# cvxopt/cvxopt

Hardware: NVIDIA H100
Metric: kkt_factor_solve_gflops_fp64 (higher is better)
Workload: dtype f64

## Files before the change

cvxopt_b200/csrc/chol.cu:

```cuda
#include "common.cuh"
#include <cstdlib>

namespace cvxb {

namespace {

constexpr int PB = 8;
constexpr int SP = 12;
constexpr int LDM = NB + 4;
constexpr int POTF2_SMEM = (NB * LDM + NB * SP + 4 * 80) * 8;
constexpr int kGroup = 4;

template <int PAT>
__device__ __forceinline__ void sym_update(double (&acc)[4][8][2], const double *Ma, const double *Mb) {
#pragma unroll 2
    for (int kk = 0; kk < NB / 4; ++kk) {
        double a[4], bfr[8];
#pragma unroll
        for (int cf = 0; cf < 4; ++cf) a[cf] = -Ma[cf * 8 + kk * 4 * LDM];
#pragma unroll
        for (int rf = 0; rf < 8; ++rf) bfr[rf] = Mb[rf * 8 + kk * 4 * LDM];
#pragma unroll
        for (int mf = 0; mf < 2; ++mf)
#pragma unroll
            for (int rf = 0; rf < 8; ++rf) {
                if (PAT == 1 && rf < 2 * mf) continue;
                if (PAT == 2 && rf < 4 + 2 * mf) continue;
                dmma16x8x4(acc[2 * mf][rf][0], acc[2 * mf][rf][1], acc[2 * mf + 1][rf][0], acc[2 * mf + 1][rf][1],
                           a[2 * mf], a[2 * mf + 1], bfr[rf]);
            }
    }
}

__global__ void __launch_bounds__(256, 1)
potf2_inv_kernel(double *A, long long lda, int jb, double *inv, double *invT, int *info, int joff,
                 long long sA, long long sInv, const double *Tprev, long long ldt,
                 const double *invprev, unsigned long long *trace) {
    extern __shared__ __align__(16) double sm[];
    if (trace && threadIdx.x == 0) {
        unsigned long long t; asm volatile("mov.u64 %0, %%globaltimer;" : "=l"(t)); trace[0] = t;
    }
#define CVXB_STAMP(SLOT)                                                                    \
    if (trace && threadIdx.x == 0) {                                                        \
        unsigned long long t_; asm volatile("mov.u64 %0, %%globaltimer;" : "=l"(t_));       \
        trace[8 * 2048 + (SLOT)] = t_;                                                      \
    }
    A += (long long)blockIdx.x * sA; inv += (long long)blockIdx.x * sInv;
    invT += (long long)blockIdx.x * sInv; info += blockIdx.x;
    double *M = sm;
    double *P = M + NB * LDM;
    double *Dw = P + NB * SP;
    const int tid = threadIdx.x, lane = tid & 31, warp = tid >> 5;
    const int role = (0x72640531 >> (warp * 4)) & 7;
    const int wr = role & 1, wc = role >> 1;
    const int g4 = lane >> 2, t4 = lane & 3;

    double acc[4][8][2];
    if (Tprev != nullptr) {
#pragma unroll
        for (int cf = 0; cf < 4; ++cf)
#pragma unroll
            for (int rf = 0; rf < 8; ++rf) acc[cf][rf][0] = acc[cf][rf][1] = 0.0;
        const int kkmax = (wc + 1) * 8;
        {
            const bool v16 = ((ldt & 1) == 0) && ((reinterpret_cast<uintptr_t>(Tprev) & 15) == 0);
            if (v16) {
                for (int q = tid; q < NB * NB / 2; q += 256) {
                    const int c = q >> 6, r = (q & 63) * 2;
                    const int nb = (r + 1 < jb) ? 16 : (r < jb ? 8 : 0);
                    cp_async16(M + r + c * LDM, nb ? Tprev + r + (long long)c * ldt : Tprev, nb);
                }
            } else {
                for (int q = tid; q < NB * NB; q += 256) {
                    const int c = q >> 7, r = q & 127;
                    cp_async8(M + r + c * LDM, (r < jb) ? Tprev + r + (long long)c * ldt : Tprev, (r < jb) ? 8 : 0);
                }
            }
            cp_async_commit();
        }
        const double *ip = invprev + (wc * 32 + g4) + t4 * NB;
        double a0[4];
#pragma unroll
        for (int cf = 0; cf < 4; ++cf) a0[cf] = ip[cf * 8];
        cp_async_wait<0>();
        __syncthreads();
        const double *tq = M + (wr * 64 + g4) + t4 * LDM;
#pragma unroll 2
        for (int kk = 0; kk < kkmax; ++kk) {
            double a[4], bfr[8];
#pragma unroll
            for (int cf = 0; cf < 4; ++cf) a[cf] = a0[cf];
            if (kk + 1 < kkmax) {
#pragma unroll
                for (int cf = 0; cf < 4; ++cf) a0[cf] = ip[cf * 8 + (kk + 1) * 4 * NB];
            }
#pragma unroll
            for (int rf = 0; rf < 8; ++rf) bfr[rf] = tq[rf * 8 + kk * 4 * LDM];
#pragma unroll
            for (int mf = 0; mf < 2; ++mf)
#pragma unroll
                for (int rf = 0; rf < 8; ++rf)
                    dmma16x8x4(acc[2 * mf][rf][0], acc[2 * mf][rf][1], acc[2 * mf + 1][rf][0],
                               acc[2 * mf + 1][rf][1], a[2 * mf], a[2 * mf + 1], bfr[rf]);
        }
        __syncthreads();
#pragma unroll
        for (int cf = 0; cf < 4; ++cf)
#pragma unroll
            for (int rf = 0; rf < 8; ++rf)
#pragma unroll
                for (int e = 0; e < 2; ++e)
                    M[(wr * 64 + rf * 8 + t4 * 2 + e) + (wc * 32 + cf * 8 + g4) * LDM] = acc[cf][rf][e];
    }
    CVXB_STAMP(0)
#pragma unroll
    for (int cf = 0; cf < 4; ++cf)
#pragma unroll
        for (int rf = 0; rf < 8; ++rf)
#pragma unroll
            for (int e = 0; e < 2; ++e) {
                const int r = wr * 64 + rf * 8 + t4 * 2 + e, c = wc * 32 + cf * 8 + g4;
                double v = (r == c) ? 1.0 : 0.0;
                if (r < jb && c < jb && r >= c) v = A[r + (long long)c * lda];
                acc[cf][rf][e] = v;
            }
    __syncthreads();
    CVXB_STAMP(4)
    if (Tprev != nullptr) {
        const int d = wc - 2 * wr;
        const double *Ma = M + (wc * 32 + g4) + t4 * LDM;
        const double *Mb = M + (wr * 64 + g4) + t4 * LDM;
        if (d < 0) sym_update<0>(acc, Ma, Mb);
        else if (d == 0) sym_update<1>(acc, Ma, Mb);
        else if (d == 1) sym_update<2>(acc, Ma, Mb);
        __syncthreads();
    }
    CVXB_STAMP(1)
#pragma unroll 1
    for (int t = 0; t < NB / PB; ++t) {
      {
        const int c0 = t * PB;
        if (wc == (t >> 2)) {
#define CVXB_PUBLISH(CF)                                                          \
    _Pragma("unroll") for (int rf = 0; rf < 8; ++rf)                              \
        _Pragma("unroll") for (int e = 0; e < 2; ++e)                             \
            P[(wr * 64 + rf * 8 + t4 * 2 + e) * SP + g4] = acc[CF][rf][e];
            switch (t & 3) {
                case 0: CVXB_PUBLISH(0) break;
                case 1: CVXB_PUBLISH(1) break;
                case 2: CVXB_PUBLISH(2) break;
                default: CVXB_PUBLISH(3) break;
            }
#undef CVXB_PUBLISH
        }
        __syncthreads();
        if (warp == 0 && lane == 0) {
            double a[PB][PB];
#pragma unroll
            for (int i = 0; i < PB; ++i)
#pragma unroll
                for (int k = 0; k <= i; ++k) a[i][k] = P[(c0 + i) * SP + k];
            bool bad = false;
#pragma unroll
            for (int j = 0; j < PB; ++j) {
                const double piv = a[j][j];
                if (!(piv > 0.0) && !bad) {
                    atomicCAS(info, 0, joff + c0 + j + 1);
                    bad = true;
                }
                const double rs = rsqrt(piv);
                a[j][j] = piv * rs;
                Dw[64 + j] = rs;
#pragma unroll
                for (int i = j + 1; i < PB; ++i) a[i][j] *= rs;
#pragma unroll
                for (int k = j + 1; k < PB; ++k)
#pragma unroll
                    for (int i = k; i < PB; ++i) a[i][k] -= a[i][j] * a[k][j];
            }
#pragma unroll
            for (int i = 0; i < PB; ++i)
#pragma unroll
                for (int k = 0; k < PB; ++k) Dw[i * 8 + k] = (k <= i) ? a[i][k] : 0.0;
        }
        if (warp < 4) asm volatile("bar.sync 1, 128;" ::: "memory");
        if (warp < 4) {
            const double *D = Dw;
            const int r = warp * 32 + lane;
            double x[PB];
            if (r >= c0 + PB) {
#pragma unroll
                for (int j = 0; j < PB; ++j) x[j] = P[r * SP + j];
#pragma unroll
                for (int j = 0; j < PB; ++j) {
                    double v = x[j];
#pragma unroll
                    for (int k = 0; k < j; ++k) v -= x[k] * D[j * 8 + k];
                    x[j] = v * D[64 + j];
                }
            } else if (r >= c0) {
#pragma unroll
                for (int j = 0; j < PB; ++j) x[j] = (j <= r - c0) ? D[(r - c0) * 8 + j] : 0.0;
            } else {
#pragma unroll
                for (int j = 0; j < PB; ++j) x[j] = 0.0;
            }
#pragma unroll
            for (int j = 0; j < PB; ++j) P[r * SP + j] = x[j];
        }
        __syncthreads();
        if (wr * 8 + 7 > t && wc * 4 + 3 > t) {
            double a[4][2], bfr[8][2];
#pragma unroll
            for (int kk = 0; kk < 2; ++kk) {
#pragma unroll
                for (int cf = 0; cf < 4; ++cf) a[cf][kk] = -P[(wc * 32 + cf * 8 + g4) * SP + kk * 4 + t4];
#pragma unroll
                for (int rf = 0; rf < 8; ++rf) bfr[rf][kk] = P[(wr * 64 + rf * 8 + g4) * SP + kk * 4 + t4];
            }
#pragma unroll
            for (int mf = 0; mf < 2; ++mf) {
                if (wc * 4 + 2 * mf + 1 <= t) continue;
#pragma unroll
                for (int rf = 0; rf < 8; ++rf) {
                    dmma16x8x4(acc[2 * mf][rf][0], acc[2 * mf][rf][1], acc[2 * mf + 1][rf][0], acc[2 * mf + 1][rf][1],
                               a[2 * mf][0], a[2 * mf + 1][0], bfr[rf][0]);
                    dmma16x8x4(acc[2 * mf][rf][0], acc[2 * mf][rf][1], acc[2 * mf + 1][rf][0], acc[2 * mf + 1][rf][1],
                               a[2 * mf][1], a[2 * mf + 1][1], bfr[rf][1]);
                }
            }
        }
        for (int e = tid; e < NB * PB; e += 256) {
            const int r = e & (NB - 1), j = e >> 7;
            const double v = P[r * SP + j];
            M[r + (c0 + j) * LDM] = v;
            if (r >= c0 + j && r < jb && c0 + j < jb) A[r + (long long)(c0 + j) * lda] = v;
        }
        __syncthreads();
      }
    }

    CVXB_STAMP(2)
    {
        const int blk = warp * 2 + (lane >> 4);
        const int j = lane & 15;
        const int o = blk * PB;
        double x[PB];
        if (j < PB) {
#pragma unroll
            for (int i = 0; i < PB; ++i) {
                double v = (i == j) ? 1.0 : 0.0;
#pragma unroll
                for (int k = 0; k < i; ++k)
                    if (k >= j) v -= M[(o + i) + (o + k) * LDM] * x[k];
                x[i] = (i >= j) ? v / M[(o + i) + (o + i) * LDM] : 0.0;
            }
        }
        __syncwarp();
        if (j < PB) {
#pragma unroll
            for (int i = 0; i < PB; ++i) M[(o + i) + (o + j) * LDM] = x[i];
        }
    }
    __syncthreads();
    for (int s = PB; s < NB; s <<= 1) {
        const int sb = s / PB;
        const int tp = sb * sb;
        const int ntiles = (NB / (2 * s)) * tp;
#pragma unroll 1
        for (int phase = 0; phase < 2; ++phase) {
            for (int base = warp * 4; base < ntiles; base += 32) {
                double c[4][2];
                int oo[4], ti[4], tj[4];
#pragma unroll
                for (int u = 0; u < 4; ++u) {
                    const int idx = min(base + u, ntiles - 1);
                    const int pr = idx / tp, loc = idx - pr * tp;
                    ti[u] = loc % sb; tj[u] = loc / sb; oo[u] = pr * 2 * s;
                    c[u][0] = c[u][1] = 0.0;
                }
                for (int kb = 0; kb < sb; ++kb) {
#pragma unroll
                    for (int u = 0; u < 4; ++u) {
                        const bool live = phase == 0 ? (kb >= tj[u]) : (kb <= ti[u]);
                        if (!live) continue;
                        const int o = oo[u];
#pragma unroll
                        for (int kk = 0; kk < 2; ++kk) {
                            const int k = kb * 8 + kk * 4 + t4;
                            double af, bf;
                            if (phase == 0) {
                                af = M[(o + s + ti[u] * 8 + g4) + (o + k) * LDM];
                                bf = M[(o + k) + (o + tj[u] * 8 + g4) * LDM];
                            } else {
                                af = M[(o + s + ti[u] * 8 + g4) + (o + s + k) * LDM];
                                bf = M[(o + k) + (o + s + tj[u] * 8 + g4) * LDM];
                            }
                            dmma(c[u][0], c[u][1], af, bf);
                        }
                    }
                }
#pragma unroll
                for (int u = 0; u < 4; ++u) {
                    if (base + u >= ntiles) continue;
                    const int o = oo[u];
                    if (phase == 0) {
                        M[(o + ti[u] * 8 + g4) + (o + s + tj[u] * 8 + t4 * 2) * LDM] = c[u][0];
                        M[(o + ti[u] * 8 + g4) + (o + s + tj[u] * 8 + t4 * 2 + 1) * LDM] = c[u][1];
                    } else {
                        M[(o + s + ti[u] * 8 + g4) + (o + tj[u] * 8 + t4 * 2) * LDM] = -c[u][0];
                        M[(o + s + ti[u] * 8 + g4) + (o + tj[u] * 8 + t4 * 2 + 1) * LDM] = -c[u][1];
                    }
                }
            }
            __syncthreads();
        }
    }
    CVXB_STAMP(3)
    for (int e = tid; e < NB * NB; e += 256) {
        int i = e & (NB - 1), k = e >> 7;
        inv[e] = (i >= k) ? M[i + k * LDM] : 0.0;
        invT[e] = (k >= i) ? M[k + i * LDM] : 0.0;
    }
    if (trace && threadIdx.x == 0) {
        unsigned long long t; asm volatile("mov.u64 %0, %%globaltimer;" : "=l"(t)); trace[1] = t;
    }
}

constexpr int TR_CH = 32;
constexpr int TR_R = 5;
constexpr int TRSV_SMEM = (TR_R * NB * TR_CH + 4 * NB + 32 * 129) * 8;

template <bool TRANS, bool VEC>
__global__ void __launch_bounds__(256, 1)
trsv_kernel(int n, const double *__restrict__ L, long long ldl, const double *__restrict__ inv,
            const double *__restrict__ invT, double *b, int *flags, int epoch, long long sL,
            long long sInv, long long sb) {
    extern __shared__ __align__(16) double sm[];
    {
        const long long pb = blockIdx.y;
        L += pb * sL; inv += pb * sInv; invT += pb * sInv; b += pb * sb;
        flags += pb * ((n + NB - 1) / NB);
    }
    double *ring = sm;
    double *xs = ring + TR_R * NB * TR_CH;
    double *part = xs + NB;
    double *tvec = part + 2 * NB;
    double *part2 = tvec + NB;
    const int nblk = (n + NB - 1) / NB;
    const int tid = threadIdx.x, lane = tid & 31, warp = tid >> 5;
    const int bi = TRANS ? (nblk - 1 - (int)blockIdx.x) : (int)blockIdx.x;
    const int i0 = bi * NB;
    const int ni = min(NB, n - i0);
    const int r = tid & (NB - 1), half = tid >> 7;

    double ireg[64];
    {
        const double *ip = (TRANS ? invT : inv) + (long long)bi * NB * NB + r + (long long)(half * 64) * NB;
#pragma unroll
        for (int k = 0; k < 64; ++k) ireg[k] = ip[k * NB];
    }

    const double bown = (tid < ni) ? b[i0 + tid] : 0.0;
    const int nb_dep = TRANS ? (nblk - 1 - bi) : bi;
    const int nchunks = nb_dep * (NB / TR_CH);
    auto issue = [&](int q) {
        const int jj = q / (NB / TR_CH), cc = q % (NB / TR_CH);
        const int j = TRANS ? (nblk - 1 - jj) : jj;
        double *dst = ring + (q % TR_R) * (NB * TR_CH);
        const double *src;
        int nrows, ncols;
        if (!TRANS) { src = L + i0 + (long long)(j * NB + cc * TR_CH) * ldl; nrows = ni; ncols = TR_CH; }
        else { src = L + (long long)j * NB + (long long)(i0 + cc * TR_CH) * ldl; nrows = min(NB, n - j * NB); ncols = min(TR_CH, ni - cc * TR_CH); }
        if (VEC) {
#pragma unroll
            for (int it = 0; it < 8; ++it) {
                const int e = tid + it * 256;
                const int c = e >> 6, rr = (e & 63) * 2;
                const int rem = nrows - rr;
                const int bytes = (c < ncols) ? (rem >= 2 ? 16 : (rem == 1 ? 8 : 0)) : 0;
                cp_async16(dst + c * NB + rr, bytes ? (src + rr + (long long)c * ldl) : L, bytes);
            }
        } else {
#pragma unroll
            for (int it = 0; it < 16; ++it) {
                const int e = tid + it * 256;
                const int c = e >> 7, rr = e & 127;
                const int bytes = (c < ncols && rr < nrows) ? 8 : 0;
                cp_async8(dst + c * NB + rr, bytes ? (src + rr + (long long)c * ldl) : L, bytes);
            }
        }
    };
#pragma unroll
    for (int q = 0; q < TR_R - 1; ++q) {
        if (q < nchunks) issue(q);
        cp_async_commit();
    }

    double acc = 0.0;
    double accc[16];
#pragma unroll
    for (int q = 0; q < 16; ++q) accc[q] = 0.0;

    for (int jj = 0; jj < nb_dep; ++jj) {
        const int j = TRANS ? (nblk - 1 - jj) : jj;
        if (tid == 0) while (ld_acquire(flags + j) != epoch) { }
        __syncthreads();
        if (tid < NB) xs[tid] = (j * NB + tid < n) ? __ldcg(b + j * NB + tid) : 0.0;
#pragma unroll
        for (int cc = 0; cc < NB / TR_CH; ++cc) {
            const int q = jj * (NB / TR_CH) + cc;
            cp_async_wait<TR_R - 2>();
            __syncthreads();
            {
                const int nq = q + TR_R - 1;
                if (nq < nchunks) issue(nq);
                cp_async_commit();
            }
            const double *ch = ring + (q % TR_R) * (NB * TR_CH);
            if (!TRANS) {
#pragma unroll
                for (int c = 0; c < 16; ++c)
                    acc += ch[(half * 16 + c) * NB + r] * xs[cc * TR_CH + half * 16 + c];
            } else {
#pragma unroll
                for (int qc = 0; qc < 4; ++qc) {
                    const double *col = ch + (warp * 4 + qc) * NB;
                    double a = 0.0;
#pragma unroll
                    for (int rr = 0; rr < 4; ++rr) a += col[lane + rr * 32] * xs[lane + rr * 32];
                    accc[cc * 4 + qc] += a;
                }
            }
        }
    }
    cp_async_wait<0>();
    __syncthreads();
    if (!TRANS) {
        part[half * NB + r] = acc;
        __syncthreads();
        if (tid < NB) tvec[tid] = (tid < ni) ? (bown - part[tid] - part[NB + tid]) : 0.0;
        __syncthreads();
    } else {
#pragma unroll
        for (int q = 0; q < 16; ++q) {
            const int c = (q >> 2) * TR_CH + warp * 4 + (q & 3);
            part2[lane * 129 + c] = accc[q];
        }
        __syncthreads();
        if (tid < NB) {
            double sacc = 0.0;
#pragma unroll 8
            for (int l = 0; l < 32; ++l) sacc += part2[l * 129 + tid];
            tvec[tid] = (tid < ni) ? (bown - sacc) : 0.0;
        }
        __syncthreads();
    }
    double a2 = 0.0;
#pragma unroll
    for (int k = 0; k < 64; ++k) a2 += ireg[k] * tvec[half * 64 + k];
    part[half * NB + r] = a2;
    __syncthreads();
    if (tid < ni) b[i0 + tid] = part[tid] + part[NB + tid];
    __threadfence();
    __syncthreads();
    if (tid == 0) st_release(flags + bi, epoch);
}

std::atomic<int> g_trsv_epoch{0};

__global__ void __launch_bounds__(256)
transpose_panel_kernel(const double *__restrict__ W, long long ldw, int rows, double *__restrict__ WT, long long ldt) {
    __shared__ double t[32][33];
    const int r0 = blockIdx.x * 32, k0 = blockIdx.y * 32, tx = threadIdx.x, ty = threadIdx.y;
#pragma unroll
    for (int i = ty; i < 32; i += 8)
        if (r0 + tx < rows) t[i][tx] = W[r0 + tx + (long long)(k0 + i) * ldw];
    __syncthreads();
#pragma unroll
    for (int i = ty; i < 32; i += 8)
        if (r0 + i < rows) WT[k0 + tx + (long long)(r0 + i) * ldt] = t[tx][i];
}

}

int chol_work_create(CholWork &w) {
    int least = 0, greatest = 0;
    CVXB_CUDA(cudaDeviceGetStreamPriorityRange(&least, &greatest));
    CVXB_CUDA(cudaStreamCreateWithPriority(&w.panel_stream, cudaStreamNonBlocking, greatest));
    CVXB_CUDA(cudaStreamCreateWithPriority(&w.trsm_stream, cudaStreamNonBlocking, greatest));
    CVXB_CUDA(cudaStreamCreateWithPriority(&w.update_stream, cudaStreamNonBlocking, least));
    CVXB_CUDA(cudaStreamCreateWithPriority(&w.near_stream, cudaStreamNonBlocking, greatest));
    CVXB_CUDA(cudaEventCreateWithFlags(&w.ev_end_t, cudaEventDisableTiming));
    CVXB_CUDA(cudaEventCreateWithFlags(&w.ev_end_n, cudaEventDisableTiming));
    CVXB_CUDA(cudaEventCreateWithFlags(&w.ev_start, cudaEventDisableTiming));
    CVXB_CUDA(cudaEventCreateWithFlags(&w.ev_end_p, cudaEventDisableTiming));
    CVXB_CUDA(cudaEventCreateWithFlags(&w.ev_end_u, cudaEventDisableTiming));
    CVXB_TRY(w.d_info.alloc(1));
    CVXB_CUDA(cudaMemset(w.d_info.p, 0, sizeof(int)));
    CVXB_TRY(w.d_flags.alloc(4096));
    CVXB_CUDA(cudaMemset(w.d_flags.p, 0, 4096 * sizeof(int)));
    CVXB_TRY(w.splitk_ws.alloc(dmma_gemm_splitk_ws_doubles()));
    CVXB_CUDA(cudaFuncSetAttribute(potf2_inv_kernel, cudaFuncAttributeMaxDynamicSharedMemorySize,
                                   POTF2_SMEM));
    CVXB_CUDA(cudaFuncSetAttribute(trsv_kernel<true, true>, cudaFuncAttributeMaxDynamicSharedMemorySize, TRSV_SMEM));
    CVXB_CUDA(cudaFuncSetAttribute(trsv_kernel<true, false>, cudaFuncAttributeMaxDynamicSharedMemorySize, TRSV_SMEM));
    CVXB_CUDA(cudaFuncSetAttribute(trsv_kernel<false, true>, cudaFuncAttributeMaxDynamicSharedMemorySize, TRSV_SMEM));
    CVXB_CUDA(cudaFuncSetAttribute(trsv_kernel<false, false>, cudaFuncAttributeMaxDynamicSharedMemorySize, TRSV_SMEM));
    return 0;
}

CholWork::~CholWork() {
    for (cudaStream_t s : {panel_stream, update_stream, trsm_stream, near_stream}) if (s) cudaStreamDestroy(s);
    for (auto &g : graphs) if (g.exec) cudaGraphExecDestroy(g.exec);
    for (cudaEvent_t e : {ev_end_t, ev_end_n, ev_start, ev_end_p, ev_end_u}) if (e) cudaEventDestroy(e);
    for (auto *v : {&ev_dg, &ev_tr, &ev_c0, &ev_na, &ev_nb, &ev_n})
        for (cudaEvent_t e : *v) cudaEventDestroy(e);
}

static int potrf_enqueue(int n, double *A, int lda, double *inv, CholWork &w, cudaStream_t st) {
    if (n <= 0) return 0;
    const int nblk = (n + NB - 1) / NB;
    if (w.panel_rows < n) {
        for (auto &g : w.graphs) if (g.exec) cudaGraphExecDestroy(g.exec);
        w.graphs.clear();
        for (DevBuf<double> &pb : w.panel) pb.reset();
        for (DevBuf<double> &gb : w.group) gb.reset();
        const int rows = (n + 1) & ~1;
        for (DevBuf<double> &pb : w.panel) CVXB_TRY(pb.alloc((size_t)rows * NB));
        for (DevBuf<double> &gb : w.group) CVXB_TRY(gb.alloc((size_t)rows * kGroup * NB));
        w.panel_rows = rows;
    }
    while ((int)w.ev_dg.size() < nblk) {
        cudaEvent_t e[6];
        for (int i = 0; i < 6; ++i) CVXB_CUDA(cudaEventCreateWithFlags(&e[i], cudaEventDisableTiming));
        w.ev_dg.push_back(e[0]); w.ev_tr.push_back(e[1]); w.ev_c0.push_back(e[2]);
        w.ev_na.push_back(e[3]); w.ev_nb.push_back(e[4]); w.ev_n.push_back(e[5]);
    }
    if (getenv("CVXB_TRACE") && !w.trace.p) CVXB_TRY(w.trace.alloc(8 * 4096));
    unsigned long long *trace = w.trace.p;
    if (trace) CVXB_CUDA(cudaMemsetAsync(trace, 0, 8 * 4096 * sizeof(unsigned long long), st));
    const int ldw = w.panel_rows;
    const int ldg = kGroup * NB;
    cudaStream_t D = w.panel_stream, T = w.trsm_stream, U = w.update_stream, N = w.near_stream;
    CVXB_CUDA(cudaMemsetAsync(w.d_info.p, 0, sizeof(int), st));
    CVXB_CUDA(cudaEventRecord(w.ev_start, st));
    for (cudaStream_t s : {D, T, U, N}) CVXB_CUDA(cudaStreamWaitEvent(s, w.ev_start, 0));
    auto update = [&](int lo, int hi, const double *X, int ldx, bool kmajor, int K, unsigned long long *tr,
                      cudaStream_t s) -> int {
        double *Acc = A + (long long)lo * NB * (1 + (long long)lda);
        GemmDesc u;
        u.M = n - lo * NB; u.N = (hi * NB < n ? hi * NB : n) - lo * NB; u.K = K;
        u.X = X; u.ldx = ldx; u.x_kmajor = kmajor;
        u.Y = X; u.ldy = ldx; u.y_kmajor = kmajor;
        u.D = Acc; u.ldd = lda; u.C = Acc; u.ldc = lda;
        u.alpha = -1.0; u.beta = 1.0; u.lower_only = true;
        u.trace = tr;
        return dmma_gemm(u, s);
    };
    auto wait_col = [&](cudaStream_t s, int c) -> int {
        const int p = c - 2, g0 = kGroup * (c / kGroup);
        if (p < 0) return 0;
        if (p >= g0) CVXB_CUDA(cudaStreamWaitEvent(s, w.ev_na[p], 0));
        if (g0 > 0) CVXB_CUDA(cudaStreamWaitEvent(s, w.ev_nb[p < g0 - 1 ? p : g0 - 1], 0));
        return 0;
    };
    for (int jb = 0; jb < nblk; ++jb) {
        const int j = jb * NB;
        const int wj = (n - j < NB) ? (n - j) : NB;
        const int m = n - j - wj;
        double *Ajj = A + j + (long long)j * lda;
        double *invj = inv + (long long)jb * NB * NB;
        double *invTj = inv + (long long)(nblk + jb) * NB * NB;
        double *Wp = w.panel[jb & 1].p;
        if (jb >= 2) CVXB_CUDA(cudaStreamWaitEvent(D, w.ev_c0[jb - 2], 0));
        CVXB_TRY(wait_col(D, jb));
        const double *Tprev = jb > 0 ? A + j + (long long)(j - NB) * lda : nullptr;
        const double *invprev = jb > 0 ? inv + (long long)(jb - 1) * NB * NB : nullptr;
        potf2_inv_kernel<<<1, 256, POTF2_SMEM, D>>>(Ajj, lda, wj, invj, invTj, w.d_info.p, j, 0, 0, Tprev,
                                                     lda, invprev, trace ? trace + 8 * jb : nullptr);
        count_launch();
        CVXB_LAUNCH_CHECK();
        CVXB_CUDA(cudaEventRecord(w.ev_dg[jb], D));
        auto copy_back_prev = [&]() -> int {
            if (jb == 0) return 0;
            const int jp = j - NB, mp = n - j;
            CVXB_CUDA(cudaMemcpy2DAsync(A + j + (long long)jp * lda, (size_t)lda * sizeof(double),
                                        w.panel[(jb - 1) & 1].p, (size_t)ldw * sizeof(double),
                                        (size_t)mp * sizeof(double), NB, cudaMemcpyDeviceToDevice, T));
            return 0;
        };
        if (m <= 0) {
            CVXB_CUDA(cudaStreamWaitEvent(T, w.ev_dg[jb], 0));
            CVXB_TRY(copy_back_prev());
            break;
        }
        double *A21 = Ajj + wj;
        double *A22 = A21 + (long long)wj * lda;
        CVXB_CUDA(cudaStreamWaitEvent(T, w.ev_dg[jb], 0));
        if (jb >= 2) CVXB_CUDA(cudaStreamWaitEvent(T, w.ev_n[jb - 2], 0));
        {
            GemmDesc g;
            g.M = m; g.N = wj; g.K = wj;
            g.X = A21; g.ldx = lda; g.x_kmajor = false;
            g.Y = invj; g.ldy = NB; g.y_kmajor = false;
            g.C = Wp; g.ldc = ldw;
            g.trace = trace ? trace + 8 * jb + 2 : nullptr;
            CVXB_TRY(dmma_gemm(g, T));
        }
        CVXB_CUDA(cudaEventRecord(w.ev_tr[jb], T));
        CVXB_TRY(wait_col(T, jb + 1));
        const int wn = (m < NB) ? m : NB;
        if (m > wn) {
            GemmDesc c;
            c.M = m - wn; c.N = wn; c.K = wj;
            c.X = Wp + wn; c.Y = Wp;
            c.ldx = ldw; c.x_kmajor = false;
            c.ldy = ldw; c.y_kmajor = false;
            c.D = A22 + wn; c.ldd = lda; c.C = A22 + wn; c.ldc = lda;
            c.alpha = -1.0; c.beta = 1.0;
            c.trace = trace ? trace + 8 * jb + 4 : nullptr;
            CVXB_TRY(dmma_gemm(c, T));
        }
        CVXB_CUDA(cudaEventRecord(w.ev_c0[jb], T));
        CVXB_TRY(copy_back_prev());
        const int q = jb / kGroup, s = jb % kGroup, gq = kGroup * (q + 1);
        double *Wg = w.group[q & 1].p;
        unsigned long long *tr_near = trace ? trace + 8 * jb + 6 : nullptr;
        CVXB_CUDA(cudaStreamWaitEvent(N, w.ev_tr[jb], 0));
        if (s == 0 && jb > 0) CVXB_CUDA(cudaStreamWaitEvent(N, w.ev_nb[jb - 1], 0));
        {
            const int lo = jb + 2, hi = gq < nblk ? gq : nblk;
            if (lo < hi) CVXB_TRY(update(lo, hi, Wp + (lo - jb - 1) * NB, ldw, false, NB, tr_near, N));
        }
        CVXB_CUDA(cudaEventRecord(w.ev_na[jb], N));
        if (gq < nblk) {
            const int rows = n - gq * NB;
            transpose_panel_kernel<<<dim3((rows + 31) / 32, NB / 32), dim3(32, 8), 0, N>>>(
                Wp + (gq - jb - 1) * NB, ldw, rows, Wg + s * NB, ldg);
            count_launch();
            CVXB_LAUNCH_CHECK();
        }
        CVXB_CUDA(cudaEventRecord(w.ev_n[jb], N));
        if (gq < nblk) {
            CVXB_CUDA(cudaStreamWaitEvent(U, w.ev_n[jb], 0));
            const int lo = gq > jb + 2 ? gq : jb + 2, hi = gq + kGroup < nblk ? gq + kGroup : nblk;
            if (lo < hi) CVXB_TRY(update(lo, hi, Wg + s * NB + (long long)(lo - gq) * NB * ldg, ldg, true, NB, tr_near, U));
            CVXB_CUDA(cudaEventRecord(w.ev_nb[jb], U));
            if (s == kGroup - 1 && gq + kGroup < nblk)
                CVXB_TRY(update(gq + kGroup, nblk, Wg + (long long)kGroup * NB * ldg, ldg, true, kGroup * NB,
                                trace ? trace + 8 * 2048 + 8 * jb + 5 : nullptr, U));
        }
    }
    CVXB_CUDA(cudaEventRecord(w.ev_end_p, D));
    CVXB_CUDA(cudaEventRecord(w.ev_end_u, U));
    CVXB_CUDA(cudaEventRecord(w.ev_end_t, T));
    CVXB_CUDA(cudaEventRecord(w.ev_end_n, N));
    for (cudaEvent_t e : {w.ev_end_p, w.ev_end_u, w.ev_end_t, w.ev_end_n}) CVXB_CUDA(cudaStreamWaitEvent(st, e, 0));
    return 0;
}

int potrf_lower(int n, double *A, int lda, double *inv, CholWork &w, cudaStream_t st) {
    if (n <= 0) return 0;
    if (w.graph_failed || n > 4096) return potrf_enqueue(n, A, lda, inv, w, st);
    CholWork::GraphEntry *ent = nullptr;
    for (auto &g : w.graphs)
        if (g.n == n && g.A == A && g.lda == lda && g.inv == inv) { ent = &g; break; }
    if (ent && ent->exec) {
        CVXB_CUDA(cudaGraphLaunch(ent->exec, st));
        count_launch(ent->launches);
        return 0;
    }
    if (!ent) {
        if (w.graphs.size() >= 4) {
            for (auto &g : w.graphs) if (g.exec) cudaGraphExecDestroy(g.exec);
            w.graphs.clear();
        }
        CholWork::GraphEntry g;
        g.n = n; g.A = A; g.lda = lda; g.inv = inv;
        w.graphs.push_back(g);
        return potrf_enqueue(n, A, lda, inv, w, st);
    }
    const unsigned long long l0 = g_launches.load();
    if (cudaStreamBeginCapture(st, cudaStreamCaptureModeRelaxed) != cudaSuccess) {
        cudaGetLastError();
        w.graph_failed = true;
        return potrf_enqueue(n, A, lda, inv, w, st);
    }
    const int rc = potrf_enqueue(n, A, lda, inv, w, st);
    cudaGraph_t graph = nullptr;
    const cudaError_t ce = cudaStreamEndCapture(st, &graph);
    const int captured = (int)(g_launches.load() - l0);
    g_launches.fetch_sub((unsigned long long)captured);
    if (rc != 0 || ce != cudaSuccess || !graph) {
        cudaGetLastError();
        if (graph) cudaGraphDestroy(graph);
        w.graph_failed = true;
        return potrf_enqueue(n, A, lda, inv, w, st);
    }
    cudaGraphExec_t exec = nullptr;
    if (cudaGraphInstantiate(&exec, graph, 0) != cudaSuccess || !exec) {
        cudaGetLastError();
        cudaGraphDestroy(graph);
        w.graph_failed = true;
        return potrf_enqueue(n, A, lda, inv, w, st);
    }
    cudaGraphDestroy(graph);
    ent->exec = exec;
    ent->launches = captured;
    CVXB_CUDA(cudaGraphLaunch(exec, st));
    count_launch(captured);
    return 0;
}

int trsv_lower(int n, const double *L, int ldl, const double *inv, double *b, bool trans,
               CholWork &w, cudaStream_t st, int batch, long long sL, long long sInv, long long sb) {
    if (n <= 0 || batch <= 0) return 0;
    const int nblk = (n + NB - 1) / NB;
    const size_t nflags = (size_t)nblk * batch;
    if (nflags > w.d_flags.n) {
        w.d_flags.reset();
        CVXB_TRY(w.d_flags.alloc(nflags));
        CVXB_CUDA(cudaMemsetAsync(w.d_flags.p, 0, nflags * sizeof(int), st));
    }
    const int epoch = g_trsv_epoch.fetch_add(1) + 1;
    const double *invT = inv + (long long)nblk * NB * NB;
    const bool vec = ((uintptr_t)L % 16 == 0) && (ldl % 2 == 0) && (batch == 1 || sL % 2 == 0);
    dim3 grid(nblk, batch);
#define TRSV_LAUNCH(T, V) trsv_kernel<T, V><<<grid, 256, TRSV_SMEM, st>>>(n, L, ldl, inv, invT, b, w.d_flags.p, epoch, sL, sInv, sb)
    if (trans) { if (vec) TRSV_LAUNCH(true, true); else TRSV_LAUNCH(true, false); }
    else       { if (vec) TRSV_LAUNCH(false, true); else TRSV_LAUNCH(false, false); }
#undef TRSV_LAUNCH
    count_launch();
    CVXB_LAUNCH_CHECK();
    return 0;
}

int potrs_lower(int n, const double *L, int ldl, const double *inv, double *b, CholWork &w,
                cudaStream_t st, int batch, long long sL, long long sInv, long long sb) {
    CVXB_TRY(trsv_lower(n, L, ldl, inv, b, false, w, st, batch, sL, sInv, sb));
    CVXB_TRY(trsv_lower(n, L, ldl, inv, b, true, w, st, batch, sL, sInv, sb));
    return 0;
}

namespace {
__global__ void copy2d_batched_kernel(const double *src, long long lds, long long ssrc, double *dst,
                                      long long ldd, long long sdst, int rows, int cols) {
    const long long pb = blockIdx.z;
    const int r = blockIdx.x * blockDim.x + threadIdx.x, c = blockIdx.y;
    if (r < rows && c < cols) dst[pb * sdst + r + (long long)c * ldd] = src[pb * ssrc + r + (long long)c * lds];
}
}

int potrf_lower_batched(int n, double *A, int lda, long long sA, double *inv, long long sInv,
                        int batch, int *d_info, double *panel, int ldw, cudaStream_t st) {
    if (n <= 0 || batch <= 0) return 0;
    const int nblk = (n + NB - 1) / NB;
    CVXB_CUDA(cudaMemsetAsync(d_info, 0, (size_t)batch * sizeof(int), st));
    const long long sW = (long long)ldw * NB;
    for (int jb = 0; jb < nblk; ++jb) {
        const int j = jb * NB;
        const int wj = (n - j < NB) ? (n - j) : NB;
        const int m = n - j - wj;
        double *Ajj = A + j + (long long)j * lda;
        double *invj = inv + (long long)jb * NB * NB;
        double *invTj = inv + (long long)(nblk + jb) * NB * NB;
        potf2_inv_kernel<<<batch, 256, POTF2_SMEM, st>>>(Ajj, lda, wj, invj, invTj, d_info, j, sA, sInv, nullptr, 0,
                                                        nullptr, nullptr);
        count_launch();
        CVXB_LAUNCH_CHECK();
        if (m <= 0) break;
        double *A21 = Ajj + wj;
        double *A22 = A21 + (long long)wj * lda;
        GemmDesc g;
        g.M = m; g.N = wj; g.K = wj;
        g.X = A21; g.ldx = lda; g.x_kmajor = false; g.sX = sA;
        g.Y = invj; g.ldy = NB; g.y_kmajor = false; g.sY = sInv;
        g.C = panel; g.ldc = ldw; g.sC = sW; g.batch = batch;
        CVXB_TRY(dmma_gemm(g, st));
        GemmDesc u;
        u.M = m; u.N = m; u.K = wj;
        u.X = panel; u.ldx = ldw; u.x_kmajor = false; u.sX = sW;
        u.Y = panel; u.ldy = ldw; u.y_kmajor = false; u.sY = sW;
        u.D = A22; u.ldd = lda; u.sD = sA; u.C = A22; u.ldc = lda; u.sC = sA;
        u.alpha = -1.0; u.beta = 1.0; u.lower_only = true; u.batch = batch;
        CVXB_TRY(dmma_gemm(u, st));
        dim3 cg((m + 255) / 256, wj, batch);
        copy2d_batched_kernel<<<cg, 256, 0, st>>>(panel, ldw, sW, A21, lda, sA, m, wj);
        count_launch();
        CVXB_LAUNCH_CHECK();
    }
    return 0;
}

}
```

cvxopt_b200/csrc/common.cuh:

```cuda
#pragma once
#include <cuda_runtime.h>
#include <cstdio>
#include <cstdint>
#include <cstring>
#include <string>
#include <vector>
#include <atomic>
#include <mutex>
#include "../../include/cvxopt_b200.h"

namespace cvxb {

void set_error(const char *fmt, ...);
extern std::atomic<unsigned long long> g_launches;
inline void count_launch(int n = 1) { g_launches.fetch_add((unsigned long long)n, std::memory_order_relaxed); }

struct DeviceOnce {
    std::atomic<unsigned long long> done{0};
    unsigned long long pending() {
        int d = 0;
        cudaGetDevice(&d);
        const unsigned long long bit = 1ull << (d & 63);
        return (done.load(std::memory_order_acquire) & bit) ? 0ull : bit;
    }
    void mark(unsigned long long bit) { done.fetch_or(bit, std::memory_order_release); }
};

#define CVXB_CUDA(expr)                                                            \
    do {                                                                           \
        cudaError_t _e = (expr);                                                   \
        if (_e != cudaSuccess) {                                                   \
            cvxb::set_error("%s:%d: %s -> %s", __FILE__, __LINE__, #expr,          \
                            cudaGetErrorString(_e));                               \
            return CVXB_E_CUDA;                                                    \
        }                                                                          \
    } while (0)

#define CVXB_TRY(expr)                                                             \
    do {                                                                           \
        int _r = (expr);                                                           \
        if (_r != 0) return _r;                                                    \
    } while (0)

#define CVXB_LAUNCH_CHECK()                                                        \
    do {                                                                           \
        cudaError_t _e = cudaGetLastError();                                       \
        if (_e != cudaSuccess) {                                                   \
            cvxb::set_error("%s:%d: kernel launch -> %s", __FILE__, __LINE__,      \
                            cudaGetErrorString(_e));                               \
            return CVXB_E_CUDA;                                                    \
        }                                                                          \
    } while (0)

cudaError_t tmp_malloc_bytes(void **p, size_t bytes);
void tmp_free(void *p);
void tmp_cache_release();
template <class T> inline cudaError_t tmp_malloc(T **p, size_t bytes) { return tmp_malloc_bytes(reinterpret_cast<void **>(p), bytes); }

template <class T> struct Scratch {
    T *p = nullptr;
    Scratch() = default;
    Scratch(const Scratch &) = delete;
    Scratch &operator=(const Scratch &) = delete;
    ~Scratch() { tmp_free(p); }
    int alloc(size_t n) {
        CVXB_CUDA(tmp_malloc(&p, (n ? n : 1) * sizeof(T)));
        return 0;
    }
};

struct Staged {
    double *dev = nullptr, *host = nullptr; size_t n = 0; bool owned = false;
    Staged() = default;
    Staged(const Staged &) = delete;
    Staged &operator=(const Staged &) = delete;
    ~Staged() { if (owned) tmp_free(dev); }
    int in(const double *src, size_t count, int space, cudaStream_t st, bool upload = true) {
        n = count; host = const_cast<double *>(src);
        if (space == CVXB_DEVICE) { dev = host; return 0; }
        CVXB_CUDA(tmp_malloc(&dev, (n ? n : 1) * sizeof(double)));
        owned = true;
        if (n && upload) CVXB_CUDA(cudaMemcpyAsync(dev, src, n * sizeof(double), cudaMemcpyHostToDevice, st));
        return 0;
    }
    int out(cudaStream_t st) {
        if (owned && n) CVXB_CUDA(cudaMemcpyAsync(host, dev, n * sizeof(double), cudaMemcpyDeviceToHost, st));
        return 0;
    }
};

extern std::atomic<unsigned long long> g_device_bytes;

template <class T> struct DevBuf {
    T *p = nullptr;
    size_t n = 0;
    DevBuf() = default;
    DevBuf(const DevBuf &) = delete;
    DevBuf &operator=(const DevBuf &) = delete;
    DevBuf(DevBuf &&o) noexcept : p(o.p), n(o.n) { o.p = nullptr; o.n = 0; }
    DevBuf &operator=(DevBuf &&o) noexcept {
        if (this != &o) { reset(); p = o.p; n = o.n; o.p = nullptr; o.n = 0; }
        return *this;
    }
    ~DevBuf() { reset(); }
    cudaError_t try_alloc(size_t count) {
        reset();
        const size_t bytes = count * sizeof(T);
        cudaError_t e = cudaMalloc(&p, bytes);
        if (e == cudaErrorMemoryAllocation) { cudaGetLastError(); tmp_cache_release(); e = cudaMalloc(&p, bytes); }
        if (e != cudaSuccess) { cudaGetLastError(); p = nullptr; return e; }
        n = count;
        g_device_bytes.fetch_add(bytes, std::memory_order_relaxed);
        return cudaSuccess;
    }
    int alloc(size_t count) {
        const cudaError_t e = try_alloc(count);
        if (e == cudaSuccess) return 0;
        set_error("cudaMalloc(%zu bytes) -> %s", count * sizeof(T), cudaGetErrorString(e));
        return e == cudaErrorMemoryAllocation ? CVXB_E_NOMEM : CVXB_E_CUDA;
    }
    void reset() {
        if (!p) return;
        cudaFree(p);
        g_device_bytes.fetch_sub(n * sizeof(T), std::memory_order_relaxed);
        p = nullptr;
        n = 0;
    }
};

bool coop_launch_fits(const void *kernel, int threads, long long ctas);

constexpr int kNumSMs = 132;
constexpr int NB = 128;

#ifdef __CUDACC__
__device__ __forceinline__ void dmma(double &d0, double &d1, double a, double b) {
    asm volatile("mma.sync.aligned.m8n8k4.row.col.f64.f64.f64.f64 {%0,%1}, {%2}, {%3}, {%0,%1};"
                 : "+d"(d0), "+d"(d1)
                 : "d"(a), "d"(b));
}
__device__ __forceinline__ void dmma16x8x4(double &d0, double &d1, double &d2, double &d3, double a0, double a1,
                                           double b) {
    asm volatile("mma.sync.aligned.m16n8k4.row.col.f64.f64.f64.f64 {%0,%1,%2,%3}, {%4,%5}, {%6}, {%0,%1,%2,%3};"
                 : "+d"(d0), "+d"(d1), "+d"(d2), "+d"(d3)
                 : "d"(a0), "d"(a1), "d"(b));
}

__device__ __forceinline__ uint32_t smem_u32(const void *p) {
    return (uint32_t)__cvta_generic_to_shared(p);
}
__device__ __forceinline__ void cp_async16(void *smem, const void *gmem, int src_bytes) {
    asm volatile("cp.async.cg.shared.global [%0], [%1], 16, %2;" ::"r"(smem_u32(smem)), "l"(gmem),
                 "r"(src_bytes));
}
__device__ __forceinline__ void cp_async8(void *smem, const void *gmem, int src_bytes) {
    asm volatile("cp.async.ca.shared.global [%0], [%1], 8, %2;" ::"r"(smem_u32(smem)), "l"(gmem),
                 "r"(src_bytes));
}
__device__ __forceinline__ void cp_async_commit() { asm volatile("cp.async.commit_group;"); }
template <int N>
__device__ __forceinline__ void cp_async_wait() {
    asm volatile("cp.async.wait_group %0;" ::"n"(N));
}

__device__ __forceinline__ void mbar_init(uint64_t *bar, int count) {
    asm volatile("mbarrier.init.shared::cta.b64 [%0], %1;" ::"r"(smem_u32(bar)), "r"(count));
}
__device__ __forceinline__ void mbar_expect_tx(uint64_t *bar, uint32_t bytes) {
    asm volatile("mbarrier.arrive.expect_tx.shared::cta.b64 _, [%0], %1;" ::"r"(smem_u32(bar)), "r"(bytes)
                 : "memory");
}
__device__ __forceinline__ void mbar_arrive(uint64_t *bar) {
    asm volatile("mbarrier.arrive.shared::cta.b64 _, [%0];" ::"r"(smem_u32(bar)) : "memory");
}
__device__ __forceinline__ void mbar_wait(uint64_t *bar, uint32_t parity) {
    asm volatile(
        "{\n\t.reg .pred p;\n\t"
        "WAIT_%=:\n\t"
        "mbarrier.try_wait.parity.shared::cta.b64 p, [%0], %1;\n\t"
        "@p bra DONE_%=;\n\t"
        "bra WAIT_%=;\n\t"
        "DONE_%=:\n\t}" ::"r"(smem_u32(bar)), "r"(parity)
        : "memory");
}
__device__ __forceinline__ void bulk_g2s(void *dst, const void *src, uint32_t bytes, uint64_t *bar) {
    asm volatile(
        "cp.async.bulk.shared::cluster.global.mbarrier::complete_tx::bytes [%0], [%1], %2, [%3];"
        ::"r"(smem_u32(dst)), "l"(src), "r"(bytes), "r"(smem_u32(bar))
        : "memory");
}
__device__ __forceinline__ void tma_load_1d(void *dst, const void *map, int c0, uint64_t *bar) {
    asm volatile(
        "cp.async.bulk.tensor.1d.shared::cluster.global.tile.mbarrier::complete_tx::bytes [%0], [%1, {%2}], [%3];"
        ::"r"(smem_u32(dst)), "l"(map), "r"(c0), "r"(smem_u32(bar))
        : "memory");
}
__device__ __forceinline__ void tma_load_2d(void *dst, const void *map, int c0, int c1, uint64_t *bar) {
    asm volatile(
        "cp.async.bulk.tensor.2d.shared::cluster.global.tile.mbarrier::complete_tx::bytes [%0], [%1, {%2, %3}], [%4];"
        ::"r"(smem_u32(dst)), "l"(map), "r"(c0), "r"(c1), "r"(smem_u32(bar))
        : "memory");
}

__device__ __forceinline__ double warp_sum(double v) {
#pragma unroll
    for (int o = 16; o > 0; o >>= 1) v += __shfl_xor_sync(0xffffffffu, v, o);
    return v;
}
__device__ __forceinline__ double warp_min(double v) {
#pragma unroll
    for (int o = 16; o > 0; o >>= 1) v = fmin(v, __shfl_xor_sync(0xffffffffu, v, o));
    return v;
}
__device__ __forceinline__ double block_sum(double v, double *sh) {
    v = warp_sum(v);
    const int lane = threadIdx.x & 31, warp = threadIdx.x >> 5;
    __syncthreads();
    if (lane == 0) sh[warp] = v;
    __syncthreads();
    double t = (threadIdx.x < (blockDim.x >> 5)) ? sh[threadIdx.x] : 0.0;
    if (warp == 0) t = warp_sum(t);
    if (threadIdx.x == 0) sh[0] = t;
    __syncthreads();
    const double r = sh[0];
    __syncthreads();
    return r;
}
__device__ __forceinline__ double block_min(double v, double *sh) {
    v = warp_min(v);
    const int lane = threadIdx.x & 31, warp = threadIdx.x >> 5;
    __syncthreads();
    if (lane == 0) sh[warp] = v;
    __syncthreads();
    double t = (threadIdx.x < (blockDim.x >> 5)) ? sh[threadIdx.x] : INFINITY;
    if (warp == 0) t = warp_min(t);
    if (threadIdx.x == 0) sh[0] = t;
    __syncthreads();
    const double r = sh[0];
    __syncthreads();
    return r;
}
__device__ __forceinline__ int ld_acquire(const int *p) {
    int v;
    asm volatile("ld.acquire.gpu.global.s32 %0, [%1];" : "=r"(v) : "l"(p) : "memory");
    return v;
}
__device__ __forceinline__ void st_release(int *p, int v) {
    asm volatile("st.release.gpu.global.s32 [%0], %1;" ::"l"(p), "r"(v) : "memory");
}
#endif

struct GemmDesc {
    int M = 0, N = 0, K = 0;
    const double *X = nullptr; int ldx = 0; bool x_kmajor = false;
    const double *Y = nullptr; int ldy = 0; bool y_kmajor = false;
    const double *w = nullptr;
    const double *D = nullptr; int ldd = 0;
    double *C = nullptr; int ldc = 0;
    double alpha = 1.0, beta = 0.0;
    bool lower_only = false;
    int ct_begin = 0, ct_end = 1 << 30;
    int batch = 1;
    long long sX = 0, sY = 0, sW = 0, sD = 0, sC = 0;
    double *splitk_ws = nullptr;
    unsigned long long *trace = nullptr;
};
int dmma_gemm(const GemmDesc &g, cudaStream_t st);
size_t dmma_gemm_splitk_ws_doubles();
int dmma_gemm_tile_cols();

size_t ozaki_workspace_bytes(int n, int m, int S);
int ozaki_mode();
bool ozaki_use(int mode, int n, int m, DevBuf<char> &work);
void ozaki_time_mma(cudaEvent_t a, cudaEvent_t b);
int ozaki_syrk(int n, int m, const double *A, long long lda, const double *d, const double *D,
               long long ldd, double beta, double *C, long long ldc, int S, int layout, void *work,
               cudaStream_t st);

struct CholWork {
    cudaStream_t panel_stream = nullptr;
    cudaStream_t trsm_stream = nullptr;
    cudaStream_t update_stream = nullptr;
    cudaStream_t near_stream = nullptr;
    cudaEvent_t ev_end_t = nullptr, ev_end_n = nullptr;
    std::vector<cudaEvent_t> ev_dg, ev_tr, ev_c0, ev_na, ev_nb, ev_n;
    DevBuf<unsigned long long> trace;
    struct GraphEntry {
        int n = 0, lda = 0, launches = 0;
        const void *A = nullptr, *inv = nullptr;
        cudaGraphExec_t exec = nullptr;
    };
    std::vector<GraphEntry> graphs;
    bool graph_failed = false;
    cudaEvent_t ev_start = nullptr, ev_end_p = nullptr, ev_end_u = nullptr;
    DevBuf<int> d_info;
    DevBuf<int> d_flags;
    DevBuf<double> splitk_ws;
    DevBuf<double> panel[2];
    DevBuf<double> group[2];
    int panel_rows = 0;
    ~CholWork();
};
int chol_work_create(CholWork &w);
int potrf_lower(int n, double *A, int lda, double *inv, CholWork &w, cudaStream_t st);
int potrs_lower(int n, const double *L, int ldl, const double *inv, double *b, CholWork &w,
                cudaStream_t st, int batch = 1, long long sL = 0, long long sInv = 0,
                long long sb = 0);
int trsv_lower(int n, const double *L, int ldl, const double *inv, double *b, bool trans,
               CholWork &w, cudaStream_t st, int batch = 1, long long sL = 0, long long sInv = 0,
               long long sb = 0);
int potrf_lower_batched(int n, double *A, int lda, long long sA, double *inv, long long sInv,
                        int batch, int *d_info, double *panel, int ldw, cudaStream_t st);
int trsm_lower_left(int n, const double *L, long long ldl, const double *inv, double *B, long long ldb, int ncols,
                    cudaStream_t st, int batch = 1, long long sL = 0, long long sInv = 0, long long sB = 0);

int check_device(int device);

struct CallCtx {
    cudaStream_t st = nullptr;
    CholWork *cw = nullptr;
    std::unique_lock<std::mutex> lock;
    int acquire(int device);
};

}
```

Measured before the change: 40640.

## Restructure blocked Cholesky lookahead so near stream covers group plus two columns

Reworks the multi-stream schedule of the blocked Cholesky factorization. The near stream now applies per-panel rank-NB updates through group boundary plus two blocks, and runs the first grouped rank-4NB update itself. The update stream only handles the far trailing matrix, using a new per-group fence event, so the panel stream waits on a single near-stream event instead of also waiting on update-stream events. This aims to take the far trailing update off the critical path, at the cost of more serial work on the near stream and trickier cross-stream dependencies.

```diff
diff --git a/cvxopt_b200/csrc/chol.cu b/cvxopt_b200/csrc/chol.cu
--- a/cvxopt_b200/csrc/chol.cu
+++ b/cvxopt_b200/csrc/chol.cu
@@ -514,7 +514,7 @@
     for (cudaStream_t s : {panel_stream, update_stream, trsm_stream, near_stream}) if (s) cudaStreamDestroy(s);
     for (auto &g : graphs) if (g.exec) cudaGraphExecDestroy(g.exec);
     for (cudaEvent_t e : {ev_end_t, ev_end_n, ev_start, ev_end_p, ev_end_u}) if (e) cudaEventDestroy(e);
-    for (auto *v : {&ev_dg, &ev_tr, &ev_c0, &ev_na, &ev_nb, &ev_n})
+    for (auto *v : {&ev_dg, &ev_tr, &ev_c0, &ev_na, &ev_n, &ev_f})
         for (cudaEvent_t e : *v) cudaEventDestroy(e);
 }
 
@@ -535,7 +535,7 @@
         cudaEvent_t e[6];
         for (int i = 0; i < 6; ++i) CVXB_CUDA(cudaEventCreateWithFlags(&e[i], cudaEventDisableTiming));
         w.ev_dg.push_back(e[0]); w.ev_tr.push_back(e[1]); w.ev_c0.push_back(e[2]);
-        w.ev_na.push_back(e[3]); w.ev_nb.push_back(e[4]); w.ev_n.push_back(e[5]);
+        w.ev_na.push_back(e[3]); w.ev_n.push_back(e[4]); w.ev_f.push_back(e[5]);
     }
     if (getenv("CVXB_TRACE") && !w.trace.p) CVXB_TRY(w.trace.alloc(8 * 4096));
     unsigned long long *trace = w.trace.p;
@@ -559,10 +559,8 @@
         return dmma_gemm(u, s);
     };
     auto wait_col = [&](cudaStream_t s, int c) -> int {
-        const int p = c - 2, g0 = kGroup * (c / kGroup);
-        if (p < 0) return 0;
-        if (p >= g0) CVXB_CUDA(cudaStreamWaitEvent(s, w.ev_na[p], 0));
-        if (g0 > 0) CVXB_CUDA(cudaStreamWaitEvent(s, w.ev_nb[p < g0 - 1 ? p : g0 - 1], 0));
+        const int p = c - 2;
+        if (p >= 0) CVXB_CUDA(cudaStreamWaitEvent(s, w.ev_na[p], 0));
         return 0;
     };
     for (int jb = 0; jb < nblk; ++jb) {
@@ -624,32 +622,33 @@
         }
         CVXB_CUDA(cudaEventRecord(w.ev_c0[jb], T));
         CVXB_TRY(copy_back_prev());
-        const int q = jb / kGroup, s = jb % kGroup, gq = kGroup * (q + 1);
+        const int q = jb / kGroup, s = jb % kGroup, g = kGroup * (q + 1);
         double *Wg = w.group[q & 1].p;
-        unsigned long long *tr_near = trace ? trace + 8 * jb + 6 : nullptr;
         CVXB_CUDA(cudaStreamWaitEvent(N, w.ev_tr[jb], 0));
-        if (s == 0 && jb > 0) CVXB_CUDA(cudaStreamWaitEvent(N, w.ev_nb[jb - 1], 0));
         {
-            const int lo = jb + 2, hi = gq < nblk ? gq : nblk;
-            if (lo < hi) CVXB_TRY(update(lo, hi, Wp + (lo - jb - 1) * NB, ldw, false, NB, tr_near, N));
+            const int lo = jb + 2, hi = g + 2 < nblk ? g + 2 : nblk;
+            if (lo < hi) CVXB_TRY(update(lo, hi, Wp + (lo - jb - 1) * NB, ldw, false, NB,
+                                         trace ? trace + 8 * jb + 6 : nullptr, N));
         }
         CVXB_CUDA(cudaEventRecord(w.ev_na[jb], N));
-        if (gq < nblk) {
-            const int rows = n - gq * NB;
+        if (g + 2 < nblk) {
+            const int rows = n - (g + 2) * NB;
             transpose_panel_kernel<<<dim3((rows + 31) / 32, NB / 32), dim3(32, 8), 0, N>>>(
-                Wp + (gq - jb - 1) * NB, ldw, rows, Wg + s * NB, ldg);
+                Wp + (g + 1 - jb) * NB, ldw, rows, Wg + s * NB, ldg);
             count_launch();
             CVXB_LAUNCH_CHECK();
         }
         CVXB_CUDA(cudaEventRecord(w.ev_n[jb], N));
-        if (gq < nblk) {
-            CVXB_CUDA(cudaStreamWaitEvent(U, w.ev_n[jb], 0));
-            const int lo = gq > jb + 2 ? gq : jb + 2, hi = gq + kGroup < nblk ? gq + kGroup : nblk;
-            if (lo < hi) CVXB_TRY(update(lo, hi, Wg + s * NB + (long long)(lo - gq) * NB * ldg, ldg, true, NB, tr_near, U));
-            CVXB_CUDA(cudaEventRecord(w.ev_nb[jb], U));
-            if (s == kGroup - 1 && gq + kGroup < nblk)
-                CVXB_TRY(update(gq + kGroup, nblk, Wg + (long long)kGroup * NB * ldg, ldg, true, kGroup * NB,
+        if (s == kGroup - 1 && g + 2 < nblk) {
+            if (q > 0) CVXB_CUDA(cudaStreamWaitEvent(N, w.ev_f[jb - kGroup], 0));
+            CVXB_TRY(update(g + 2, g + 2 + kGroup < nblk ? g + 2 + kGroup : nblk, Wg, ldg, true, kGroup * NB, nullptr,
+                            N));
+            if (g + 2 + kGroup < nblk) {
+                CVXB_CUDA(cudaStreamWaitEvent(U, w.ev_n[jb], 0));
+                CVXB_TRY(update(g + 2 + kGroup, nblk, Wg + (long long)kGroup * NB * ldg, ldg, true, kGroup * NB,
                                 trace ? trace + 8 * 2048 + 8 * jb + 5 : nullptr, U));
+            }
+            CVXB_CUDA(cudaEventRecord(w.ev_f[jb], U));
         }
     }
     CVXB_CUDA(cudaEventRecord(w.ev_end_p, D));
diff --git a/cvxopt_b200/csrc/common.cuh b/cvxopt_b200/csrc/common.cuh
--- a/cvxopt_b200/csrc/common.cuh
+++ b/cvxopt_b200/csrc/common.cuh
@@ -283,7 +283,7 @@
     cudaStream_t update_stream = nullptr;
     cudaStream_t near_stream = nullptr;
     cudaEvent_t ev_end_t = nullptr, ev_end_n = nullptr;
-    std::vector<cudaEvent_t> ev_dg, ev_tr, ev_c0, ev_na, ev_nb, ev_n;
+    std::vector<cudaEvent_t> ev_dg, ev_tr, ev_c0, ev_na, ev_n, ev_f;
     DevBuf<unsigned long long> trace;
     struct GraphEntry {
         int n = 0, lda = 0, launches = 0;
```

New measurement: 41050, median of 6. 1.01x the previous value.
